# showlab/VideoSwap

Hardware: NVIDIA H100
Metric: denoise-steps/sec, 16f 512^2 SD1.5 UNet3D (CFG UNet fwd + CFG combine + DDIM step) (higher is better)
Workload: dtype f16

## Files before the change

videoswap_b200/csrc/attention_tc.cu:

```cuda
#include "common.cuh"
#include "kernels.h"

namespace vs {
namespace {

constexpr int TQ = 64;
constexpr int ATT_THREADS = 384;
constexpr int PRODUCER_REGS = 24, CONSUMER_REGS = 240;

template <int D>
struct TCfg {
  static constexpr int BKV = 128;
  static constexpr int STAGES = D > 64 ? 3 : 4;
  static constexpr int NCB = (D + 63) / 64;
  static constexpr int DPK = (D + 15) / 16 * 16;
  static constexpr int Q_BLOCK = TQ * 128;
  static constexpr int KV_BLOCK = BKV * 128;
  static constexpr int Q_BYTES = NCB * Q_BLOCK;
  static constexpr int KV_STAGE_BYTES = 2 * NCB * KV_BLOCK;
  static constexpr int OREG = (D > 64) ? 32 + 8 : 32;
  static constexpr int SMEM = 2 * Q_BYTES + STAGES * KV_STAGE_BYTES + 1024 + 8 * (1 + 2 * STAGES);
  static_assert(D == 40 || D == 80, "head dims of the tensor-core path");
  static_assert(SMEM <= 227 * 1024, "shared memory");
};

struct TAttnArgs {
  CUtensorMap tmQ, tmK, tmV;
  __half* o;
  int ldo;
  long long o_bs;
  int nq, nk, kv_div;
  float scale_log2;
};

__device__ __forceinline__ float fast_exp2(float x) {
  float y;
  asm("ex2.approx.ftz.f32 %0, %1;" : "=f"(y) : "f"(x));
  return y;
}
__device__ __forceinline__ uint32_t pack_h2(float a, float b) {
  const __half2 h = __floats2half2_rn(a, b);
  return *reinterpret_cast<const uint32_t*>(&h);
}

template <int D>
__global__ void __launch_bounds__(ATT_THREADS, 1) attn_tc_kernel(const __grid_constant__ TAttnArgs p) {
  using C = TCfg<D>;
  constexpr int BKV = C::BKV, STAGES = C::STAGES;
  extern __shared__ uint8_t smem_raw[];
  const uint32_t base = (smem_u32(smem_raw) + 1023u) & ~1023u;
  const uint32_t q_s = base;
  const uint32_t kv_s = q_s + 2 * C::Q_BYTES;
  const uint32_t bars = kv_s + STAGES * C::KV_STAGE_BYTES;
  const uint32_t q_full = bars;
  auto kv_full = [&](int s) { return bars + 8u * (1 + s); };
  auto kv_empty = [&](int s) { return bars + 8u * (1 + STAGES + s); };

  const int warp = threadIdx.x >> 5, lane = threadIdx.x & 31, wg = threadIdx.x >> 7;
  const int q0 = blockIdx.x * 2 * TQ, head = blockIdx.y, b = blockIdx.z;
  const int nkt = (p.nk + BKV - 1) / BKV;

  if (threadIdx.x == 0) {
    prefetch_tmap(&p.tmQ); prefetch_tmap(&p.tmK); prefetch_tmap(&p.tmV);
    mbar_init(q_full, 1);
    for (int s = 0; s < STAGES; ++s) {
      mbar_init(kv_full(s), 1);
      mbar_init(kv_empty(s), 8);
    }
    fence_barrier_init();
  }
  __syncthreads();
  pdl_trigger();
  pdl_wait();

  if (wg == 0) {
    setmaxnreg_dec<PRODUCER_REGS>();
    if (warp != 0) return;
    const int bk = b / p.kv_div;
    if (elect_one()) {
      mbar_expect_tx(q_full, 2 * C::Q_BYTES);
#pragma unroll
      for (int g = 0; g < 2; ++g)
#pragma unroll
        for (int cb = 0; cb < C::NCB; ++cb)
          tma_load_4d(q_s + g * C::Q_BYTES + cb * C::Q_BLOCK, &p.tmQ, q_full, cb * 64, head, q0 + g * TQ, b);
    }
    __syncwarp();
    for (int j = 0, s = 0, ph = 0; j < nkt; ++j) {
      mbar_wait(kv_empty(s), ph ^ 1);
      if (elect_one()) {
        const uint32_t k_dst = kv_s + s * C::KV_STAGE_BYTES, v_dst = k_dst + C::NCB * C::KV_BLOCK;
        mbar_expect_tx(kv_full(s), C::KV_STAGE_BYTES);
#pragma unroll
        for (int cb = 0; cb < C::NCB; ++cb) {
          tma_load_4d(k_dst + cb * C::KV_BLOCK, &p.tmK, kv_full(s), cb * 64, head, j * BKV, bk);
          tma_load_4d(v_dst + cb * C::KV_BLOCK, &p.tmV, kv_full(s), cb * 64, head, j * BKV, bk);
        }
      }
      __syncwarp();
      if (++s == STAGES) { s = 0; ph ^= 1; }
    }
    return;
  }

  setmaxnreg_inc<CONSUMER_REGS>();
  const int g = wg - 1, wq = warp & 3, q4 = lane & 3;
  const uint32_t qg = q_s + g * C::Q_BYTES;
  const int bar_mine = 1 + g, bar_other = 2 - g;
  if (g == 1) named_bar_arrive(bar_other, 256);

  const float sc = p.scale_log2;
  float o[C::OREG];
#pragma unroll
  for (int i = 0; i < C::OREG; ++i) o[i] = 0.f;
  float m[2] = {-INFINITY, -INFINITY}, l[2] = {0.f, 0.f};
  float s[BKV / 2];
  uint32_t pf[BKV / 16][4];

  auto stage_addr = [&](int j) { return kv_s + (uint32_t)(j % STAGES) * C::KV_STAGE_BYTES; };
  auto issue_qk = [&](int j) {
    const uint32_t k_a = stage_addr(j);
#pragma unroll
    for (int k = 0; k < C::DPK / 16; ++k) {
      const uint32_t qoff = (uint32_t)((k * 16) / 64) * C::Q_BLOCK + (uint32_t)((k * 16) % 64) * 2;
      const uint32_t koff = (uint32_t)((k * 16) / 64) * C::KV_BLOCK + (uint32_t)((k * 16) % 64) * 2;
      wgmma_ss<BKV>(s, gmma_desc_sw128(qg + qoff), gmma_desc_sw128(k_a + koff), k != 0 ? 1u : 0u);
    }
  };
  auto issue_pv = [&](int j) {
    const uint32_t v_a = stage_addr(j) + C::NCB * C::KV_BLOCK;
#pragma unroll
    for (int kk = 0; kk < BKV / 16; ++kk) {
      const uint32_t v_rows = v_a + kk * 16 * 128;
      wgmma_m64n64_rs<1>(o, pf[kk], gmma_desc_sw128_mn(v_rows, C::KV_BLOCK), 1u);
      if (D > 64) wgmma_m64n16_rs<1>(o + 32, pf[kk], gmma_desc_sw128_mn(v_rows + C::KV_BLOCK, C::KV_BLOCK), 1u);
    }
  };
  auto softmax = [&](int j, float* alpha) {
    const int kbase = j * BKV;
    if (kbase + BKV > p.nk) {
#pragma unroll
      for (int i = 0; i < BKV / 2; ++i)
        if (kbase + 8 * (i >> 2) + 2 * q4 + (i & 1) >= p.nk) s[i] = -INFINITY;
    }
#pragma unroll
    for (int h = 0; h < 2; ++h) {
      float mx = m[h];
#pragma unroll
      for (int i = 2 * h; i < BKV / 2; i += 4) mx = fmaxf(mx, fmaxf(s[i], s[i + 1]));
      mx = fmaxf(mx, __shfl_xor_sync(0xffffffffu, mx, 1));
      mx = fmaxf(mx, __shfl_xor_sync(0xffffffffu, mx, 2));
      alpha[h] = fast_exp2((m[h] - mx) * sc);
      m[h] = mx;
      const float ms = mx * sc;
      float rs = 0.f;
#pragma unroll
      for (int i = 2 * h; i < BKV / 2; i += 4) {
        s[i] = fast_exp2(fmaf(s[i], sc, -ms));
        s[i + 1] = fast_exp2(fmaf(s[i + 1], sc, -ms));
        rs += s[i] + s[i + 1];
      }
      l[h] = fmaf(l[h], alpha[h], rs);
    }
  };
  auto pack_p = [&]() {
#pragma unroll
    for (int kk = 0; kk < BKV / 16; ++kk)
#pragma unroll
      for (int r = 0; r < 4; ++r) pf[kk][r] = pack_h2(s[8 * kk + 2 * r], s[8 * kk + 2 * r + 1]);
  };
  auto release = [&](int j) {
    if (lane == 0) mbar_arrive(kv_empty(j % STAGES));
  };

  mbar_wait(q_full, 0);
  mbar_wait(kv_full(0), 0);
  named_bar_sync(bar_mine, 256);
  wgmma_fence();
  issue_qk(0);
  wgmma_commit();
  named_bar_arrive(bar_other, 256);
  wgmma_wait<0>();
  {
    float alpha[2];
    softmax(0, alpha);
    pack_p();
  }
  for (int j = 1; j < nkt; ++j) {
    mbar_wait(kv_full(j % STAGES), (j / STAGES) & 1);
    named_bar_sync(bar_mine, 256);
    wgmma_fence();
    issue_qk(j);
    wgmma_commit();
    issue_pv(j - 1);
    wgmma_commit();
    named_bar_arrive(bar_other, 256);
    wgmma_wait<1>();
    float alpha[2];
    softmax(j, alpha);
    if (p.kv_div > 0) wgmma_wait<0>();
    release(j - 1);
#pragma unroll
    for (int i = 0; i < C::OREG; ++i) o[i] *= alpha[(i >> 1) & 1];
    pack_p();
  }
  named_bar_sync(bar_mine, 256);
  wgmma_fence();
  issue_pv(nkt - 1);
  wgmma_commit();
  if (g == 0) named_bar_arrive(bar_other, 256);
  wgmma_wait<0>();
  release(nkt - 1);

#pragma unroll
  for (int h = 0; h < 2; ++h) {
    l[h] += __shfl_xor_sync(0xffffffffu, l[h], 1);
    l[h] += __shfl_xor_sync(0xffffffffu, l[h], 2);
  }
  const float inv[2] = {1.f / l[0], 1.f / l[1]};
  const int r0 = q0 + g * TQ + 16 * wq + (lane >> 2);
  __half* ob = p.o + b * p.o_bs + head * D;
#pragma unroll
  for (int i = 0; i < C::OREG; i += 2) {
    const int h = (i >> 1) & 1, c = 8 * (i >> 2) + 2 * q4, r = r0 + 8 * h;
    if (c < D && r < p.nq)
      *reinterpret_cast<__half2*>(ob + (long long)r * p.ldo + c) = __floats2half2_rn(o[i] * inv[h], o[i + 1] * inv[h]);
  }
}

template <int D>
int launch(cudaStream_t st, const __half* q, int ldq, const __half* k, int ldk, const __half* v, int ldv, __half* o, int ldo,
           int batch, int nq, int nk, int heads, long long q_bs, long long kv_bs, long long o_bs, int kv_div) {
  using C = TCfg<D>;
  static bool configured = false;
  if (!configured) {
    VS_CHECK_CUDA(cudaFuncSetAttribute(attn_tc_kernel<D>, cudaFuncAttributeMaxDynamicSharedMemorySize, C::SMEM));
    configured = true;
  }
  TAttnArgs a;
  memset(&a, 0, sizeof(a));
  const int bkv = (batch + kv_div - 1) / kv_div;
  {
    const uint64_t dims[4] = {(uint64_t)D, (uint64_t)heads, (uint64_t)nq, (uint64_t)batch};
    const uint64_t str[3] = {(uint64_t)D * 2, (uint64_t)ldq * 2, (uint64_t)(q_bs > 0 ? q_bs : (long long)nq * ldq) * 2};
    const uint32_t box[4] = {64, 1, TQ, 1};
    if (make_tmap_f16(&a.tmQ, q, 4, dims, str, box, 1)) return 3;
  }
  {
    const uint64_t dims[4] = {(uint64_t)D, (uint64_t)heads, (uint64_t)nk, (uint64_t)bkv};
    const uint64_t strk[3] = {(uint64_t)D * 2, (uint64_t)ldk * 2, (uint64_t)(kv_bs > 0 ? kv_bs : (long long)nk * ldk) * 2};
    const uint64_t strv[3] = {(uint64_t)D * 2, (uint64_t)ldv * 2, (uint64_t)(kv_bs > 0 ? kv_bs : (long long)nk * ldv) * 2};
    const uint32_t box[4] = {64, 1, (uint32_t)C::BKV, 1};
    if (make_tmap_f16(&a.tmK, k, 4, dims, strk, box, 1)) return 3;
    if (make_tmap_f16(&a.tmV, v, 4, dims, strv, box, 1)) return 3;
  }
  a.o = o; a.ldo = ldo; a.o_bs = o_bs; a.nq = nq; a.nk = nk; a.kv_div = kv_div;
  a.scale_log2 = 1.4426950408889634f / sqrtf((float)D);
  ProfScope prof(st, PC_ATTN, 4.0 * batch * heads * (double)nq * nk * D, 1, nq, nk, D);
  dim3 grid((nq + 2 * TQ - 1) / (2 * TQ), heads, batch);
  return launch_pdl(attn_tc_kernel<D>, grid, dim3(ATT_THREADS), C::SMEM, st, 1, a);
}

}

int attention_tc(cudaStream_t st, const __half* q, int ldq, const __half* k, int ldk, const __half* v, int ldv, __half* o,
                 int ldo, int batch, int nq, int nk, int heads, int d, long long q_bs, long long kv_bs, long long o_bs,
                 int kv_div) {
  if ((ldq % 8) || (ldk % 8) || (ldv % 8) || (ldo % 2)) return -1;
  if ((q_bs % 8) || (kv_bs % 8)) return -1;
  VS_REQUIRE(kv_div >= 1, "attention_tc: kv_div must be >= 1 (got %d)", kv_div);
  if (d == 40) return launch<40>(st, q, ldq, k, ldk, v, ldv, o, ldo, batch, nq, nk, heads, q_bs, kv_bs, o_bs, kv_div);
  if (d == 80) return launch<80>(st, q, ldq, k, ldk, v, ldv, o, ldo, batch, nq, nk, heads, q_bs, kv_bs, o_bs, kv_div);
  return -1;
}

}
```

videoswap_b200/csrc/common.cuh:

```cuda
#pragma once
#include <cuda.h>
#include <cuda_fp16.h>
#include <cuda_runtime.h>
#include <stdint.h>
#include <stdio.h>

namespace vs {

void set_error(const char* fmt, ...);
const char* last_error();

#define VS_CHECK_CUDA(expr)                                                                         \
  do {                                                                                              \
    cudaError_t _e = (expr);                                                                        \
    if (_e != cudaSuccess) {                                                                        \
      vs::set_error("%s:%d CUDA error %s: %s", __FILE__, __LINE__, #expr, cudaGetErrorString(_e)); \
      return 1;                                                                                     \
    }                                                                                               \
  } while (0)

#define VS_REQUIRE(cond, ...)                \
  do {                                       \
    if (!(cond)) {                           \
      vs::set_error(__VA_ARGS__);            \
      return 2;                              \
    }                                        \
  } while (0)

int make_tmap_f16(CUtensorMap* out, const void* base, int rank, const uint64_t* dims, const uint64_t* strides_bytes,
                  const uint32_t* box, int swizzle );

int num_sms();
int get_option(const char* name);

#ifdef __CUDACC__
template <typename... KArgs, typename... Args>
int launch_pdl(void (*kernel)(KArgs...), dim3 grid, dim3 block, size_t smem, cudaStream_t st, int cluster_x, Args&&... args) {
  cudaLaunchConfig_t cfg = {};
  cfg.gridDim = grid;
  cfg.blockDim = block;
  cfg.dynamicSmemBytes = smem;
  cfg.stream = st;
  cudaLaunchAttribute attr[2];
  int n = 0;
  if (get_option("pdl") != 0) {
    attr[n].id = cudaLaunchAttributeProgrammaticStreamSerialization;
    attr[n].val.programmaticStreamSerializationAllowed = 1;
    ++n;
  }
  if (cluster_x > 1) {
    attr[n].id = cudaLaunchAttributeClusterDimension;
    attr[n].val.clusterDim.x = cluster_x;
    attr[n].val.clusterDim.y = 1;
    attr[n].val.clusterDim.z = 1;
    ++n;
  }
  cfg.attrs = attr;
  cfg.numAttrs = n;
  VS_CHECK_CUDA(cudaLaunchKernelEx(&cfg, kernel, static_cast<KArgs>(args)...));
  return 0;
}
#endif

enum ProfCat { PC_GEMM = 0, PC_CONV = 1, PC_ATTN = 2, PC_TATTN = 3, PC_GROUPNORM = 4, PC_LAYERNORM = 5, PC_OTHER = 6, PC_COUNT = 7 };
struct ProfScope {
  ProfScope(cudaStream_t st, int cat, double work, int nlaunch = 1, long long m = 0, int n = 0, int k = 0);
  ~ProfScope();
  cudaStream_t st_; int idx_;
};
void prof_enable(bool on);
void prof_reset();
int prof_collect(int cat, double* ms, double* work, long long* count);
int prof_dump(const char* path);
long long launch_count();
void count_launch(int n);

#ifdef __CUDACC__
__device__ __forceinline__ uint32_t smem_u32(const void* p) { return (uint32_t)__cvta_generic_to_shared(p); }

__device__ __forceinline__ void mbar_init(uint32_t bar, uint32_t count) {
  asm volatile("mbarrier.init.shared::cta.b64 [%0], %1;" ::"r"(bar), "r"(count) : "memory");
}
__device__ __forceinline__ void fence_barrier_init() {
  asm volatile("fence.mbarrier_init.release.cluster;" ::: "memory");
}
__device__ __forceinline__ void fence_proxy_async() { asm volatile("fence.proxy.async.shared::cta;" ::: "memory"); }
__device__ __forceinline__ void mbar_expect_tx(uint32_t bar, uint32_t bytes) {
  asm volatile("mbarrier.arrive.expect_tx.shared::cta.b64 _, [%0], %1;" ::"r"(bar), "r"(bytes) : "memory");
}
__device__ __forceinline__ void mbar_arrive(uint32_t bar) {
  asm volatile("mbarrier.arrive.shared::cta.b64 _, [%0];" ::"r"(bar) : "memory");
}
__device__ __forceinline__ bool mbar_try_wait(uint32_t bar, uint32_t parity) {
  uint32_t ok;
  asm volatile(
      "{\n\t.reg .pred p;\n\t"
      "mbarrier.try_wait.parity.shared::cta.b64 p, [%1], %2;\n\t"
      "selp.u32 %0, 1, 0, p;\n\t}"
      : "=r"(ok)
      : "r"(bar), "r"(parity)
      : "memory");
  return ok != 0;
}
__device__ __forceinline__ void mbar_wait(uint32_t bar, uint32_t parity) {
  if (mbar_try_wait(bar, parity)) return;
  uint32_t spins = 0;
  while (!mbar_try_wait(bar, parity)) {
    if (++spins > (1u << 25)) __trap();
  }
}

__device__ __forceinline__ void prefetch_tmap(const CUtensorMap* m) {
  asm volatile("prefetch.tensormap [%0];" ::"l"(reinterpret_cast<uint64_t>(m)) : "memory");
}
__device__ __forceinline__ void tma_load_2d(uint32_t dst, const CUtensorMap* m, uint32_t bar, int c0, int c1) {
  asm volatile(
      "cp.async.bulk.tensor.2d.shared::cluster.global.mbarrier::complete_tx::bytes [%0], [%1, {%3, %4}], [%2];"
      ::"r"(dst), "l"(reinterpret_cast<uint64_t>(m)), "r"(bar), "r"(c0), "r"(c1)
      : "memory");
}
__device__ __forceinline__ void bulk_load(uint32_t dst, const void* src, uint32_t bytes, uint32_t bar) {
  asm volatile(
      "cp.async.bulk.shared::cluster.global.mbarrier::complete_tx::bytes [%0], [%1], %2, [%3];"
      ::"r"(dst), "l"(reinterpret_cast<uint64_t>(src)), "r"(bytes), "r"(bar)
      : "memory");
}
__device__ __forceinline__ void tma_load_4d(uint32_t dst, const CUtensorMap* m, uint32_t bar, int c0, int c1, int c2,
                                            int c3) {
  asm volatile(
      "cp.async.bulk.tensor.4d.shared::cluster.global.mbarrier::complete_tx::bytes [%0], [%1, {%3, %4, %5, %6}], [%2];"
      ::"r"(dst), "l"(reinterpret_cast<uint64_t>(m)), "r"(bar), "r"(c0), "r"(c1), "r"(c2), "r"(c3)
      : "memory");
}

__device__ __forceinline__ bool elect_one() {
  uint32_t pred;
  asm volatile(
      "{\n\t.reg .pred P;\n\t"
      "elect.sync _|P, 0xffffffff;\n\t"
      "selp.u32 %0, 1, 0, P;\n\t}"
      : "=r"(pred));
  return pred != 0;
}

__device__ __forceinline__ uint32_t cluster_ctarank() {
  uint32_t r;
  asm volatile("mov.u32 %0, %%cluster_ctarank;" : "=r"(r));
  return r;
}
__device__ __forceinline__ void cluster_sync_all() {
  asm volatile("barrier.cluster.arrive.release.aligned;" ::: "memory");
  asm volatile("barrier.cluster.wait.acquire.aligned;" ::: "memory");
}
__device__ __forceinline__ uint32_t mapa_shared(uint32_t addr, uint32_t rank) {
  uint32_t r;
  asm volatile("mapa.shared::cluster.u32 %0, %1, %2;" : "=r"(r) : "r"(addr), "r"(rank));
  return r;
}
__device__ __forceinline__ void named_bar_sync(int id, int nthreads) {
  asm volatile("bar.sync %0, %1;" ::"r"(id), "r"(nthreads) : "memory");
}
__device__ __forceinline__ void named_bar_arrive(int id, int nthreads) {
  asm volatile("bar.arrive %0, %1;" ::"r"(id), "r"(nthreads) : "memory");
}

__device__ __forceinline__ void pdl_trigger() { asm volatile("griddepcontrol.launch_dependents;" ::: "memory"); }
__device__ __forceinline__ void pdl_wait() { asm volatile("griddepcontrol.wait;" ::: "memory"); }

template <int N>
__device__ __forceinline__ void setmaxnreg_dec() { asm volatile("setmaxnreg.dec.sync.aligned.u32 %0;" ::"n"(N)); }
template <int N>
__device__ __forceinline__ void setmaxnreg_inc() { asm volatile("setmaxnreg.inc.sync.aligned.u32 %0;" ::"n"(N)); }

__device__ __forceinline__ void wgmma_fence() { asm volatile("wgmma.fence.sync.aligned;" ::: "memory"); }
__device__ __forceinline__ void wgmma_commit() { asm volatile("wgmma.commit_group.sync.aligned;" ::: "memory"); }
template <int N>
__device__ __forceinline__ void wgmma_wait() { asm volatile("wgmma.wait_group.sync.aligned %0;" ::"n"(N) : "memory"); }

__device__ __forceinline__ uint64_t gmma_desc_sw128(uint32_t smem_addr) {
  uint64_t d = 0;
  d |= (uint64_t)((smem_addr & 0x3FFFF) >> 4);
  d |= (uint64_t)1 << 16;
  d |= (uint64_t)(1024 >> 4) << 32;
  d |= (uint64_t)1 << 62;
  return d;
}
__device__ __forceinline__ uint64_t gmma_desc_sw128_mn(uint32_t smem_addr, uint32_t lbo_bytes) {
  uint64_t d = 0;
  d |= (uint64_t)((smem_addr & 0x3FFFF) >> 4);
  d |= (uint64_t)((lbo_bytes >> 4) & 0x3FFF) << 16;
  d |= (uint64_t)(1024 >> 4) << 32;
  d |= (uint64_t)1 << 62;
  return d;
}

#define VS_R8(i) "+f"(d[i]), "+f"(d[i + 1]), "+f"(d[i + 2]), "+f"(d[i + 3]), "+f"(d[i + 4]), "+f"(d[i + 5]), "+f"(d[i + 6]), "+f"(d[i + 7])
template <int N>
__device__ __forceinline__ void wgmma_ss(float* d, uint64_t da, uint64_t db, uint32_t scale_d);
#define VS_REGS_0_31 "%0,%1,%2,%3,%4,%5,%6,%7,%8,%9,%10,%11,%12,%13,%14,%15,%16,%17,%18,%19,%20,%21,%22,%23,%24,%25,%26,%27,%28,%29,%30,%31"
#define VS_REGS_32_63 "%32,%33,%34,%35,%36,%37,%38,%39,%40,%41,%42,%43,%44,%45,%46,%47,%48,%49,%50,%51,%52,%53,%54,%55,%56,%57,%58,%59,%60,%61,%62,%63"
#define VS_REGS_64_79 "%64,%65,%66,%67,%68,%69,%70,%71,%72,%73,%74,%75,%76,%77,%78,%79"
#define VS_REGS_80_127 "%80,%81,%82,%83,%84,%85,%86,%87,%88,%89,%90,%91,%92,%93,%94,%95,%96,%97,%98,%99,%100,%101,%102,%103,%104,%105,%106,%107,%108,%109,%110,%111,%112,%113,%114,%115,%116,%117,%118,%119,%120,%121,%122,%123,%124,%125,%126,%127"
#define VS_WGMMA_SS(N, REGS, IA, IB, IS, ...)                                                                     \
  template <>                                                                                                     \
  __device__ __forceinline__ void wgmma_ss<N>(float* d, uint64_t da, uint64_t db, uint32_t scale_d) {           \
    asm volatile("{\n\t.reg .pred p;\n\tsetp.ne.b32 p, %" #IS ", 0;\n\t"                                         \
                 "wgmma.mma_async.sync.aligned.m64n" #N "k16.f32.f16.f16 {" REGS "}, %" #IA ", %" #IB ", p, 1, 1, 0, 0;\n\t}" \
                 : __VA_ARGS__                                                                                    \
                 : "l"(da), "l"(db), "r"(scale_d));                                                               \
  }
VS_WGMMA_SS(64, VS_REGS_0_31, 32, 33, 34, VS_R8(0), VS_R8(8), VS_R8(16), VS_R8(24))
VS_WGMMA_SS(128, VS_REGS_0_31 "," VS_REGS_32_63, 64, 65, 66, VS_R8(0), VS_R8(8), VS_R8(16), VS_R8(24), VS_R8(32), VS_R8(40),
            VS_R8(48), VS_R8(56))
VS_WGMMA_SS(160, VS_REGS_0_31 "," VS_REGS_32_63 "," VS_REGS_64_79, 80, 81, 82, VS_R8(0), VS_R8(8), VS_R8(16), VS_R8(24),
            VS_R8(32), VS_R8(40), VS_R8(48), VS_R8(56), VS_R8(64), VS_R8(72))
VS_WGMMA_SS(256, VS_REGS_0_31 "," VS_REGS_32_63 "," VS_REGS_64_79 "," VS_REGS_80_127, 128, 129, 130, VS_R8(0), VS_R8(8),
            VS_R8(16), VS_R8(24), VS_R8(32), VS_R8(40), VS_R8(48), VS_R8(56), VS_R8(64), VS_R8(72), VS_R8(80), VS_R8(88),
            VS_R8(96), VS_R8(104), VS_R8(112), VS_R8(120))
#undef VS_WGMMA_SS
#undef VS_REGS_0_31
#undef VS_REGS_32_63
#undef VS_REGS_64_79
#undef VS_REGS_80_127
template <int TB = 0>
__device__ __forceinline__ void wgmma_m64n16(float* d, uint64_t da, uint64_t db, uint32_t scale_d) {
  asm volatile(
      "{\n\t.reg .pred p;\n\tsetp.ne.b32 p, %10, 0;\n\t"
      "wgmma.mma_async.sync.aligned.m64n16k16.f32.f16.f16 {%0,%1,%2,%3,%4,%5,%6,%7}, %8, %9, p, 1, 1, 0, %11;\n\t}"
      : VS_R8(0)
      : "l"(da), "l"(db), "r"(scale_d), "n"(TB));
}
template <int TB = 0>
__device__ __forceinline__ void wgmma_m64n64_rs(float* d, const uint32_t* a, uint64_t db, uint32_t scale_d) {
  asm volatile(
      "{\n\t.reg .pred p;\n\tsetp.ne.b32 p, %37, 0;\n\t"
      "wgmma.mma_async.sync.aligned.m64n64k16.f32.f16.f16 "
      "{%0,%1,%2,%3,%4,%5,%6,%7,%8,%9,%10,%11,%12,%13,%14,%15,%16,%17,%18,%19,%20,%21,%22,%23,%24,%25,%26,%27,%28,%29,%30,%31}, "
      "{%32,%33,%34,%35}, %36, p, 1, 1, %38;\n\t}"
      : VS_R8(0), VS_R8(8), VS_R8(16), VS_R8(24)
      : "r"(a[0]), "r"(a[1]), "r"(a[2]), "r"(a[3]), "l"(db), "r"(scale_d), "n"(TB));
}
template <int TB = 0>
__device__ __forceinline__ void wgmma_m64n16_rs(float* d, const uint32_t* a, uint64_t db, uint32_t scale_d) {
  asm volatile(
      "{\n\t.reg .pred p;\n\tsetp.ne.b32 p, %13, 0;\n\t"
      "wgmma.mma_async.sync.aligned.m64n16k16.f32.f16.f16 {%0,%1,%2,%3,%4,%5,%6,%7}, {%8,%9,%10,%11}, %12, p, 1, 1, %14;\n\t}"
      : VS_R8(0)
      : "r"(a[0]), "r"(a[1]), "r"(a[2]), "r"(a[3]), "l"(db), "r"(scale_d), "n"(TB));
}
#undef VS_R8

__device__ __forceinline__ float silu_f(float x) { return __fdividef(x, 1.f + __expf(-x)); }
__device__ __forceinline__ float gelu_erf_f(float x) { return 0.5f * x * (1.f + erff(x * 0.70710678118654752f)); }
__device__ __forceinline__ float gelu_erf_fast(float x) {
  const float z = fabsf(x) * 0.70710678118654752f;
  float t;
  asm("rcp.approx.ftz.f32 %0, %1;" : "=f"(t) : "f"(fmaf(0.3275911f, z, 1.f)));
  float poly = fmaf(1.061405429f, t, -1.453152027f);
  poly = fmaf(poly, t, 1.421413741f);
  poly = fmaf(poly, t, -0.284496736f);
  poly = fmaf(poly, t, 0.254829592f);
  poly *= t;
  float e;
  asm("ex2.approx.ftz.f32 %0, %1;" : "=f"(e) : "f"(-1.4426950408889634f * z * z));
  const float erf_abs = fmaf(-poly, e, 1.f);
  const float erf_s = copysignf(erf_abs, x);
  return 0.5f * x * (1.f + erf_s);
}
__device__ __forceinline__ float gelu_sig(float x) {
  const float xn = fmaxf(x, -5.f);
  const float xc = fminf(xn, 5.f);
  const float u = xc * xc;
  float q = fmaf(u, 2.47135360e-05f, 7.37690930e-04f);
  q = fmaf(q, u, -1.05988323e-01f);
  q = fmaf(q, u, -2.30164247e+00f);
  float e;
  asm("ex2.approx.ftz.f32 %0, %1;" : "=f"(e) : "f"(xc * q));
  return __fdividef(xn, 1.f + e);
}
__device__ __forceinline__ float quick_gelu_f(float v) {
  const float t = fminf(-2.4554669595930157f * v, 64.f);
  float e;
  asm("ex2.approx.ftz.f32 %0, %1;" : "=f"(e) : "f"(t));
  return __fdividef(v, 1.f + e);
}
#endif

}
```

Measured before the change: 11.35.

## Make tensor-core attention persistent and use exact-width n40 PV wgmma

Converts the attention kernel into a persistent kernel: the grid is capped at the SM count and each CTA loops over (q-block, head, batch) work items. A new q_empty barrier lets the producer prefetch the next item's Q and K/V while the consumers finish the current one, and the stage index carries across items. For head dim 40, the PV product now uses a single m64n40 wgmma instead of an n64 one, which drops padded columns and their accumulator registers. The aim is to hide launch and tail costs and overlap item boundaries, at the price of more complex barrier phase tracking and possible load imbalance.

```diff
diff --git a/videoswap_b200/csrc/attention_tc.cu b/videoswap_b200/csrc/attention_tc.cu
--- a/videoswap_b200/csrc/attention_tc.cu
+++ b/videoswap_b200/csrc/attention_tc.cu
@@ -1,5 +1,13 @@
 #include "common.cuh"
 #include "kernels.h"
+
+#include <algorithm>
+
+#ifndef VS_ATTN_PHASE
+#define VS_ATTN_PHASE(k)
+#define VS_ATTN_PHASES_BEGIN
+#define VS_ATTN_PHASES_END
+#endif
 
 namespace vs {
 namespace {
@@ -18,8 +26,8 @@
   static constexpr int KV_BLOCK = BKV * 128;
   static constexpr int Q_BYTES = NCB * Q_BLOCK;
   static constexpr int KV_STAGE_BYTES = 2 * NCB * KV_BLOCK;
-  static constexpr int OREG = (D > 64) ? 32 + 8 : 32;
-  static constexpr int SMEM = 2 * Q_BYTES + STAGES * KV_STAGE_BYTES + 1024 + 8 * (1 + 2 * STAGES);
+  static constexpr int OREG = D / 2;
+  static constexpr int SMEM = 2 * Q_BYTES + STAGES * KV_STAGE_BYTES + 1024 + 8 * (2 + 2 * STAGES);
   static_assert(D == 40 || D == 80, "head dims of the tensor-core path");
   static_assert(SMEM <= 227 * 1024, "shared memory");
 };
@@ -30,6 +38,7 @@
   int ldo;
   long long o_bs;
   int nq, nk, kv_div;
+  int heads, nqb, items;
   float scale_log2;
 };
 
@@ -52,17 +61,23 @@
   const uint32_t q_s = base;
   const uint32_t kv_s = q_s + 2 * C::Q_BYTES;
   const uint32_t bars = kv_s + STAGES * C::KV_STAGE_BYTES;
-  const uint32_t q_full = bars;
-  auto kv_full = [&](int s) { return bars + 8u * (1 + s); };
-  auto kv_empty = [&](int s) { return bars + 8u * (1 + STAGES + s); };
+  const uint32_t q_full = bars, q_empty = bars + 8u;
+  auto kv_full = [&](int s) { return bars + 8u * (2 + s); };
+  auto kv_empty = [&](int s) { return bars + 8u * (2 + STAGES + s); };
 
   const int warp = threadIdx.x >> 5, lane = threadIdx.x & 31, wg = threadIdx.x >> 7;
-  const int q0 = blockIdx.x * 2 * TQ, head = blockIdx.y, b = blockIdx.z;
   const int nkt = (p.nk + BKV - 1) / BKV;
+  auto item = [&](int w, int& q0, int& head, int& b) {
+    const int hb = w / p.nqb;
+    q0 = (w - hb * p.nqb) * 2 * TQ;
+    head = hb % p.heads;
+    b = hb / p.heads;
+  };
 
   if (threadIdx.x == 0) {
     prefetch_tmap(&p.tmQ); prefetch_tmap(&p.tmK); prefetch_tmap(&p.tmV);
     mbar_init(q_full, 1);
+    mbar_init(q_empty, 8);
     for (int s = 0; s < STAGES; ++s) {
       mbar_init(kv_full(s), 1);
       mbar_init(kv_empty(s), 8);
@@ -76,34 +91,41 @@
   if (wg == 0) {
     setmaxnreg_dec<PRODUCER_REGS>();
     if (warp != 0) return;
-    const int bk = b / p.kv_div;
-    if (elect_one()) {
-      mbar_expect_tx(q_full, 2 * C::Q_BYTES);
-#pragma unroll
-      for (int g = 0; g < 2; ++g)
-#pragma unroll
-        for (int cb = 0; cb < C::NCB; ++cb)
-          tma_load_4d(q_s + g * C::Q_BYTES + cb * C::Q_BLOCK, &p.tmQ, q_full, cb * 64, head, q0 + g * TQ, b);
-    }
-    __syncwarp();
-    for (int j = 0, s = 0, ph = 0; j < nkt; ++j) {
-      mbar_wait(kv_empty(s), ph ^ 1);
+    int s = 0, ph = 0;
+    for (int w = blockIdx.x, it = 0; w < p.items; w += gridDim.x, ++it) {
+      int q0, head, b;
+      item(w, q0, head, b);
+      const int bk = b / p.kv_div;
+      if (it > 0) mbar_wait(q_empty, (it - 1) & 1);
       if (elect_one()) {
-        const uint32_t k_dst = kv_s + s * C::KV_STAGE_BYTES, v_dst = k_dst + C::NCB * C::KV_BLOCK;
-        mbar_expect_tx(kv_full(s), C::KV_STAGE_BYTES);
-#pragma unroll
-        for (int cb = 0; cb < C::NCB; ++cb) {
-          tma_load_4d(k_dst + cb * C::KV_BLOCK, &p.tmK, kv_full(s), cb * 64, head, j * BKV, bk);
-          tma_load_4d(v_dst + cb * C::KV_BLOCK, &p.tmV, kv_full(s), cb * 64, head, j * BKV, bk);
-        }
+        mbar_expect_tx(q_full, 2 * C::Q_BYTES);
+#pragma unroll
+        for (int g = 0; g < 2; ++g)
+#pragma unroll
+          for (int cb = 0; cb < C::NCB; ++cb)
+            tma_load_4d(q_s + g * C::Q_BYTES + cb * C::Q_BLOCK, &p.tmQ, q_full, cb * 64, head, q0 + g * TQ, b);
       }
       __syncwarp();
-      if (++s == STAGES) { s = 0; ph ^= 1; }
+      for (int j = 0; j < nkt; ++j) {
+        mbar_wait(kv_empty(s), ph ^ 1);
+        if (elect_one()) {
+          const uint32_t k_dst = kv_s + s * C::KV_STAGE_BYTES, v_dst = k_dst + C::NCB * C::KV_BLOCK;
+          mbar_expect_tx(kv_full(s), C::KV_STAGE_BYTES);
+#pragma unroll
+          for (int cb = 0; cb < C::NCB; ++cb) {
+            tma_load_4d(k_dst + cb * C::KV_BLOCK, &p.tmK, kv_full(s), cb * 64, head, j * BKV, bk);
+            tma_load_4d(v_dst + cb * C::KV_BLOCK, &p.tmV, kv_full(s), cb * 64, head, j * BKV, bk);
+          }
+        }
+        __syncwarp();
+        if (++s == STAGES) { s = 0; ph ^= 1; }
+      }
     }
     return;
   }
 
   setmaxnreg_inc<CONSUMER_REGS>();
+  VS_ATTN_PHASES_BEGIN;
   const int g = wg - 1, wq = warp & 3, q4 = lane & 3;
   const uint32_t qg = q_s + g * C::Q_BYTES;
   const int bar_mine = 1 + g, bar_other = 2 - g;
@@ -111,13 +133,12 @@
 
   const float sc = p.scale_log2;
   float o[C::OREG];
-#pragma unroll
-  for (int i = 0; i < C::OREG; ++i) o[i] = 0.f;
-  float m[2] = {-INFINITY, -INFINITY}, l[2] = {0.f, 0.f};
+  float m[2], l[2];
   float s[BKV / 2];
   uint32_t pf[BKV / 16][4];
-
-  auto stage_addr = [&](int j) { return kv_s + (uint32_t)(j % STAGES) * C::KV_STAGE_BYTES; };
+  int t0 = 0;
+
+  auto stage_addr = [&](int j) { return kv_s + (uint32_t)((t0 + j) % STAGES) * C::KV_STAGE_BYTES; };
   auto issue_qk = [&](int j) {
     const uint32_t k_a = stage_addr(j);
 #pragma unroll
@@ -132,8 +153,12 @@
 #pragma unroll
     for (int kk = 0; kk < BKV / 16; ++kk) {
       const uint32_t v_rows = v_a + kk * 16 * 128;
-      wgmma_m64n64_rs<1>(o, pf[kk], gmma_desc_sw128_mn(v_rows, C::KV_BLOCK), 1u);
-      if (D > 64) wgmma_m64n16_rs<1>(o + 32, pf[kk], gmma_desc_sw128_mn(v_rows + C::KV_BLOCK, C::KV_BLOCK), 1u);
+      if constexpr (D == 40) {
+        wgmma_m64n40_rs<1>(o, pf[kk], gmma_desc_sw128_mn(v_rows, C::KV_BLOCK), 1u);
+      } else {
+        wgmma_m64n64_rs<1>(o, pf[kk], gmma_desc_sw128_mn(v_rows, C::KV_BLOCK), 1u);
+        wgmma_m64n16_rs<1>(o + 32, pf[kk], gmma_desc_sw128_mn(v_rows + C::KV_BLOCK, C::KV_BLOCK), 1u);
+      }
     }
   };
   auto softmax = [&](int j, float* alpha) {
@@ -150,6 +175,7 @@
       for (int i = 2 * h; i < BKV / 2; i += 4) mx = fmaxf(mx, fmaxf(s[i], s[i + 1]));
       mx = fmaxf(mx, __shfl_xor_sync(0xffffffffu, mx, 1));
       mx = fmaxf(mx, __shfl_xor_sync(0xffffffffu, mx, 2));
+      VS_ATTN_PHASE(4);
       alpha[h] = fast_exp2((m[h] - mx) * sc);
       m[h] = mx;
       const float ms = mx * sc;
@@ -161,6 +187,7 @@
         rs += s[i] + s[i + 1];
       }
       l[h] = fmaf(l[h], alpha[h], rs);
+      VS_ATTN_PHASE(5);
     }
   };
   auto pack_p = [&]() {
@@ -170,62 +197,88 @@
       for (int r = 0; r < 4; ++r) pf[kk][r] = pack_h2(s[8 * kk + 2 * r], s[8 * kk + 2 * r + 1]);
   };
   auto release = [&](int j) {
-    if (lane == 0) mbar_arrive(kv_empty(j % STAGES));
-  };
-
-  mbar_wait(q_full, 0);
-  mbar_wait(kv_full(0), 0);
-  named_bar_sync(bar_mine, 256);
-  wgmma_fence();
-  issue_qk(0);
-  wgmma_commit();
-  named_bar_arrive(bar_other, 256);
-  wgmma_wait<0>();
-  {
-    float alpha[2];
-    softmax(0, alpha);
-    pack_p();
-  }
-  for (int j = 1; j < nkt; ++j) {
-    mbar_wait(kv_full(j % STAGES), (j / STAGES) & 1);
+    if (lane == 0) mbar_arrive(kv_empty((t0 + j) % STAGES));
+  };
+  auto kv_wait = [&](int j) { mbar_wait(kv_full((t0 + j) % STAGES), ((t0 + j) / STAGES) & 1); };
+  auto q_release = [&]() {
+    if (lane == 0) mbar_arrive(q_empty);
+  };
+
+  for (int w = blockIdx.x, it = 0; w < p.items; w += gridDim.x, ++it, t0 += nkt) {
+    int q0, head, b;
+    item(w, q0, head, b);
+    const bool last_item = w + (int)gridDim.x >= p.items;
+#pragma unroll
+    for (int i = 0; i < C::OREG; ++i) o[i] = 0.f;
+    m[0] = m[1] = -INFINITY;
+    l[0] = l[1] = 0.f;
+
+    mbar_wait(q_full, it & 1);
+    kv_wait(0);
     named_bar_sync(bar_mine, 256);
     wgmma_fence();
-    issue_qk(j);
-    wgmma_commit();
-    issue_pv(j - 1);
+    issue_qk(0);
     wgmma_commit();
     named_bar_arrive(bar_other, 256);
-    wgmma_wait<1>();
-    float alpha[2];
-    softmax(j, alpha);
-    if (p.kv_div > 0) wgmma_wait<0>();
-    release(j - 1);
-#pragma unroll
-    for (int i = 0; i < C::OREG; ++i) o[i] *= alpha[(i >> 1) & 1];
-    pack_p();
-  }
-  named_bar_sync(bar_mine, 256);
-  wgmma_fence();
-  issue_pv(nkt - 1);
-  wgmma_commit();
-  if (g == 0) named_bar_arrive(bar_other, 256);
-  wgmma_wait<0>();
-  release(nkt - 1);
-
-#pragma unroll
-  for (int h = 0; h < 2; ++h) {
-    l[h] += __shfl_xor_sync(0xffffffffu, l[h], 1);
-    l[h] += __shfl_xor_sync(0xffffffffu, l[h], 2);
-  }
-  const float inv[2] = {1.f / l[0], 1.f / l[1]};
-  const int r0 = q0 + g * TQ + 16 * wq + (lane >> 2);
-  __half* ob = p.o + b * p.o_bs + head * D;
-#pragma unroll
-  for (int i = 0; i < C::OREG; i += 2) {
-    const int h = (i >> 1) & 1, c = 8 * (i >> 2) + 2 * q4, r = r0 + 8 * h;
-    if (c < D && r < p.nq)
-      *reinterpret_cast<__half2*>(ob + (long long)r * p.ldo + c) = __floats2half2_rn(o[i] * inv[h], o[i + 1] * inv[h]);
-  }
+    wgmma_wait<0>();
+    if (nkt == 1) q_release();
+    VS_ATTN_PHASE(8);
+    {
+      float alpha[2];
+      softmax(0, alpha);
+      pack_p();
+    }
+    for (int j = 1; j < nkt; ++j) {
+      kv_wait(j);
+      VS_ATTN_PHASE(0);
+      named_bar_sync(bar_mine, 256);
+      VS_ATTN_PHASE(1);
+      wgmma_fence();
+      issue_qk(j);
+      wgmma_commit();
+      issue_pv(j - 1);
+      wgmma_commit();
+      named_bar_arrive(bar_other, 256);
+      VS_ATTN_PHASE(2);
+      wgmma_wait<1>();
+      if (j == nkt - 1) q_release();
+      VS_ATTN_PHASE(3);
+      float alpha[2];
+      softmax(j, alpha);
+      if (p.kv_div > 0) wgmma_wait<0>();
+      release(j - 1);
+      VS_ATTN_PHASE(6);
+#pragma unroll
+      for (int i = 0; i < C::OREG; ++i) o[i] *= alpha[(i >> 1) & 1];
+      pack_p();
+      VS_ATTN_PHASE(7);
+    }
+    named_bar_sync(bar_mine, 256);
+    wgmma_fence();
+    issue_pv(nkt - 1);
+    wgmma_commit();
+    if (g == 0 || !last_item) named_bar_arrive(bar_other, 256);
+    wgmma_wait<0>();
+    release(nkt - 1);
+
+#pragma unroll
+    for (int h = 0; h < 2; ++h) {
+      l[h] += __shfl_xor_sync(0xffffffffu, l[h], 1);
+      l[h] += __shfl_xor_sync(0xffffffffu, l[h], 2);
+    }
+    const float inv[2] = {1.f / l[0], 1.f / l[1]};
+    const int r0 = q0 + g * TQ + 16 * wq + (lane >> 2);
+    __half* ob = p.o + b * p.o_bs + head * D;
+#pragma unroll
+    for (int i = 0; i < C::OREG; i += 2) {
+      const int h = (i >> 1) & 1, c = 8 * (i >> 2) + 2 * q4, r = r0 + 8 * h;
+      if (c < D && r < p.nq)
+        *reinterpret_cast<__half2*>(ob + (long long)r * p.ldo + c) =
+            __floats2half2_rn(o[i] * inv[h], o[i + 1] * inv[h]);
+    }
+    VS_ATTN_PHASE(8);
+  }
+  VS_ATTN_PHASES_END;
 }
 
 template <int D>
@@ -255,9 +308,12 @@
     if (make_tmap_f16(&a.tmV, v, 4, dims, strv, box, 1)) return 3;
   }
   a.o = o; a.ldo = ldo; a.o_bs = o_bs; a.nq = nq; a.nk = nk; a.kv_div = kv_div;
+  a.heads = heads;
+  a.nqb = (nq + 2 * TQ - 1) / (2 * TQ);
+  a.items = a.nqb * heads * batch;
   a.scale_log2 = 1.4426950408889634f / sqrtf((float)D);
   ProfScope prof(st, PC_ATTN, 4.0 * batch * heads * (double)nq * nk * D, 1, nq, nk, D);
-  dim3 grid((nq + 2 * TQ - 1) / (2 * TQ), heads, batch);
+  const dim3 grid(std::min(a.items, num_sms()));
   return launch_pdl(attn_tc_kernel<D>, grid, dim3(ATT_THREADS), C::SMEM, st, 1, a);
 }
 
diff --git a/videoswap_b200/csrc/common.cuh b/videoswap_b200/csrc/common.cuh
--- a/videoswap_b200/csrc/common.cuh
+++ b/videoswap_b200/csrc/common.cuh
@@ -238,6 +238,15 @@
       "{%0,%1,%2,%3,%4,%5,%6,%7,%8,%9,%10,%11,%12,%13,%14,%15,%16,%17,%18,%19,%20,%21,%22,%23,%24,%25,%26,%27,%28,%29,%30,%31}, "
       "{%32,%33,%34,%35}, %36, p, 1, 1, %38;\n\t}"
       : VS_R8(0), VS_R8(8), VS_R8(16), VS_R8(24)
+      : "r"(a[0]), "r"(a[1]), "r"(a[2]), "r"(a[3]), "l"(db), "r"(scale_d), "n"(TB));
+}
+template <int TB = 0>
+__device__ __forceinline__ void wgmma_m64n40_rs(float* d, const uint32_t* a, uint64_t db, uint32_t scale_d) {
+  asm volatile(
+      "{\n\t.reg .pred p;\n\tsetp.ne.b32 p, %25, 0;\n\t"
+      "wgmma.mma_async.sync.aligned.m64n40k16.f32.f16.f16 "
+      "{%0,%1,%2,%3,%4,%5,%6,%7,%8,%9,%10,%11,%12,%13,%14,%15,%16,%17,%18,%19}, {%20,%21,%22,%23}, %24, p, 1, 1, %26;\n\t}"
+      : VS_R8(0), VS_R8(8), "+f"(d[16]), "+f"(d[17]), "+f"(d[18]), "+f"(d[19])
       : "r"(a[0]), "r"(a[1]), "r"(a[2]), "r"(a[3]), "l"(db), "r"(scale_d), "n"(TB));
 }
 template <int TB = 0>
```

After: 11.48 (median of 6 runs). 1.2% higher.

## Use three consumer warpgroups for head dim 40 attention with ping-pong rotation

Applied to the files above, without the earlier changes.

For head dim 40 the tensor-core attention kernel now runs three consumer warpgroups per CTA (lower register cap of 160) instead of two, so each CTA covers 192 query rows and reuses every K/V stage across more queries. The named-barrier ping-pong is generalized to a round-robin ring, and warpgroups whose query tile is out of range still join the barrier and release protocol. mbarrier waits switch to a spin loop with no trap guard, and a __nanosleep is added in the kv_div<=0 branch. Risks include register spills at 160 registers, fewer CTAs, and loss of hang detection.

```diff
diff --git a/videoswap_b200/csrc/attention_tc.cu b/videoswap_b200/csrc/attention_tc.cu
--- a/videoswap_b200/csrc/attention_tc.cu
+++ b/videoswap_b200/csrc/attention_tc.cu
@@ -5,13 +5,15 @@
 namespace {
 
 constexpr int TQ = 64;
-constexpr int ATT_THREADS = 384;
-constexpr int PRODUCER_REGS = 24, CONSUMER_REGS = 240;
+constexpr int PRODUCER_REGS = 24;
 
 template <int D>
 struct TCfg {
   static constexpr int BKV = 128;
   static constexpr int STAGES = D > 64 ? 3 : 4;
+  static constexpr int NCONS = D > 64 ? 2 : 3;
+  static constexpr int THREADS = 128 * (1 + NCONS);
+  static constexpr int CONSUMER_REGS = D > 64 ? 240 : 160;
   static constexpr int NCB = (D + 63) / 64;
   static constexpr int DPK = (D + 15) / 16 * 16;
   static constexpr int Q_BLOCK = TQ * 128;
@@ -19,9 +21,10 @@
   static constexpr int Q_BYTES = NCB * Q_BLOCK;
   static constexpr int KV_STAGE_BYTES = 2 * NCB * KV_BLOCK;
   static constexpr int OREG = (D > 64) ? 32 + 8 : 32;
-  static constexpr int SMEM = 2 * Q_BYTES + STAGES * KV_STAGE_BYTES + 1024 + 8 * (1 + 2 * STAGES);
+  static constexpr int SMEM = NCONS * Q_BYTES + STAGES * KV_STAGE_BYTES + 1024 + 8 * (1 + 2 * STAGES);
   static_assert(D == 40 || D == 80, "head dims of the tensor-core path");
   static_assert(SMEM <= 227 * 1024, "shared memory");
+  static_assert(128 * PRODUCER_REGS + 128 * NCONS * CONSUMER_REGS <= 64 * 1024, "register file");
 };
 
 struct TAttnArgs {
@@ -44,20 +47,20 @@
 }
 
 template <int D>
-__global__ void __launch_bounds__(ATT_THREADS, 1) attn_tc_kernel(const __grid_constant__ TAttnArgs p) {
+__global__ void __launch_bounds__(TCfg<D>::THREADS, 1) attn_tc_kernel(const __grid_constant__ TAttnArgs p) {
   using C = TCfg<D>;
-  constexpr int BKV = C::BKV, STAGES = C::STAGES;
+  constexpr int BKV = C::BKV, STAGES = C::STAGES, NCONS = C::NCONS;
   extern __shared__ uint8_t smem_raw[];
   const uint32_t base = (smem_u32(smem_raw) + 1023u) & ~1023u;
   const uint32_t q_s = base;
-  const uint32_t kv_s = q_s + 2 * C::Q_BYTES;
+  const uint32_t kv_s = q_s + NCONS * C::Q_BYTES;
   const uint32_t bars = kv_s + STAGES * C::KV_STAGE_BYTES;
   const uint32_t q_full = bars;
   auto kv_full = [&](int s) { return bars + 8u * (1 + s); };
   auto kv_empty = [&](int s) { return bars + 8u * (1 + STAGES + s); };
 
   const int warp = threadIdx.x >> 5, lane = threadIdx.x & 31, wg = threadIdx.x >> 7;
-  const int q0 = blockIdx.x * 2 * TQ, head = blockIdx.y, b = blockIdx.z;
+  const int q0 = blockIdx.x * NCONS * TQ, head = blockIdx.y, b = blockIdx.z;
   const int nkt = (p.nk + BKV - 1) / BKV;
 
   if (threadIdx.x == 0) {
@@ -65,7 +68,7 @@
     mbar_init(q_full, 1);
     for (int s = 0; s < STAGES; ++s) {
       mbar_init(kv_full(s), 1);
-      mbar_init(kv_empty(s), 8);
+      mbar_init(kv_empty(s), 4 * NCONS);
     }
     fence_barrier_init();
   }
@@ -78,9 +81,9 @@
     if (warp != 0) return;
     const int bk = b / p.kv_div;
     if (elect_one()) {
-      mbar_expect_tx(q_full, 2 * C::Q_BYTES);
-#pragma unroll
-      for (int g = 0; g < 2; ++g)
+      mbar_expect_tx(q_full, NCONS * C::Q_BYTES);
+#pragma unroll
+      for (int g = 0; g < NCONS; ++g)
 #pragma unroll
         for (int cb = 0; cb < C::NCB; ++cb)
           tma_load_4d(q_s + g * C::Q_BYTES + cb * C::Q_BLOCK, &p.tmQ, q_full, cb * 64, head, q0 + g * TQ, b);
@@ -103,11 +106,22 @@
     return;
   }
 
-  setmaxnreg_inc<CONSUMER_REGS>();
+  setmaxnreg_inc<C::CONSUMER_REGS>();
   const int g = wg - 1, wq = warp & 3, q4 = lane & 3;
   const uint32_t qg = q_s + g * C::Q_BYTES;
-  const int bar_mine = 1 + g, bar_other = 2 - g;
-  if (g == 1) named_bar_arrive(bar_other, 256);
+  const int bar_mine = 1 + g, bar_next = 1 + (g + 1) % NCONS;
+  const bool last_cons = g == NCONS - 1;
+  if (last_cons) named_bar_arrive(bar_next, 256);
+
+  if (q0 + g * TQ >= p.nq) {
+    for (int j = 0; j <= nkt; ++j) {
+      if (j < nkt) mbar_wait_spin(kv_full(j % STAGES), (j / STAGES) & 1);
+      named_bar_sync(bar_mine, 256);
+      if (j < nkt || !last_cons) named_bar_arrive(bar_next, 256);
+      if (j > 0 && lane == 0) mbar_arrive(kv_empty((j - 1) % STAGES));
+    }
+    return;
+  }
 
   const float sc = p.scale_log2;
   float o[C::OREG];
@@ -173,13 +187,13 @@
     if (lane == 0) mbar_arrive(kv_empty(j % STAGES));
   };
 
-  mbar_wait(q_full, 0);
-  mbar_wait(kv_full(0), 0);
+  mbar_wait_spin(q_full, 0);
+  mbar_wait_spin(kv_full(0), 0);
   named_bar_sync(bar_mine, 256);
   wgmma_fence();
   issue_qk(0);
   wgmma_commit();
-  named_bar_arrive(bar_other, 256);
+  named_bar_arrive(bar_next, 256);
   wgmma_wait<0>();
   {
     float alpha[2];
@@ -187,18 +201,23 @@
     pack_p();
   }
   for (int j = 1; j < nkt; ++j) {
-    mbar_wait(kv_full(j % STAGES), (j / STAGES) & 1);
+    mbar_wait_spin(kv_full(j % STAGES), (j / STAGES) & 1);
     named_bar_sync(bar_mine, 256);
     wgmma_fence();
     issue_qk(j);
     wgmma_commit();
     issue_pv(j - 1);
     wgmma_commit();
-    named_bar_arrive(bar_other, 256);
+    named_bar_arrive(bar_next, 256);
     wgmma_wait<1>();
     float alpha[2];
     softmax(j, alpha);
-    if (p.kv_div > 0) wgmma_wait<0>();
+    if (p.kv_div > 0) {
+      wgmma_wait<0>();
+    } else {
+      wgmma_wait<0>();
+      __nanosleep(32);
+    }
     release(j - 1);
 #pragma unroll
     for (int i = 0; i < C::OREG; ++i) o[i] *= alpha[(i >> 1) & 1];
@@ -208,7 +227,7 @@
   wgmma_fence();
   issue_pv(nkt - 1);
   wgmma_commit();
-  if (g == 0) named_bar_arrive(bar_other, 256);
+  if (!last_cons) named_bar_arrive(bar_next, 256);
   wgmma_wait<0>();
   release(nkt - 1);
 
@@ -257,8 +276,8 @@
   a.o = o; a.ldo = ldo; a.o_bs = o_bs; a.nq = nq; a.nk = nk; a.kv_div = kv_div;
   a.scale_log2 = 1.4426950408889634f / sqrtf((float)D);
   ProfScope prof(st, PC_ATTN, 4.0 * batch * heads * (double)nq * nk * D, 1, nq, nk, D);
-  dim3 grid((nq + 2 * TQ - 1) / (2 * TQ), heads, batch);
-  return launch_pdl(attn_tc_kernel<D>, grid, dim3(ATT_THREADS), C::SMEM, st, 1, a);
+  dim3 grid((nq + C::NCONS * TQ - 1) / (C::NCONS * TQ), heads, batch);
+  return launch_pdl(attn_tc_kernel<D>, grid, dim3(C::THREADS), C::SMEM, st, 1, a);
 }
 
 }
diff --git a/videoswap_b200/csrc/common.cuh b/videoswap_b200/csrc/common.cuh
--- a/videoswap_b200/csrc/common.cuh
+++ b/videoswap_b200/csrc/common.cuh
@@ -107,6 +107,10 @@
   uint32_t spins = 0;
   while (!mbar_try_wait(bar, parity)) {
     if (++spins > (1u << 25)) __trap();
+  }
+}
+__device__ __forceinline__ void mbar_wait_spin(uint32_t bar, uint32_t parity) {
+  while (!mbar_try_wait(bar, parity)) {
   }
 }
 
```

Measured after the change: 11.43 before, 11.68 after (median of 6 runs). 1.02x the previous value.
